# pain7576/ddpg-trucktrailer

Measured on AMD Instinct MI355X. Metric: env-steps/s, higher is better.
Workload: dtype f64

## Files before the change

### ddpg-trucktrailer_amd/_lib.py

```python
import ctypes as C
import os

HERE = os.path.dirname(os.path.abspath(__file__))
LIB_PATH = os.environ.get("TT_LIB_PATH") or os.path.join(HERE, "libttenv.so")

OBS_DIM = 23
MAX_EPISODE_STEPS = 4095
TT_OK, TT_EINVAL, TT_ENOMEM, TT_EHIP, TT_ENODEV = 0, -1, -2, -3, -4
F_JACKKNIFE, F_OUT_OF_MAP, F_MAX_STEPS, F_GOAL_REACHED, F_GOAL_PASSED, F_EXCESSIVE_BACK, F_SUCCESS = (1 << i for i in range(7))
VIOLATIONS = ("none", "jackknife", "jackknife_warning", "major_boundary", "minor_boundary", "past_the_goal",
              "max_step", "excessive_backward")
INFO_ROWS = ("total_reward", "progress_reward", "heading_reward", "orientation_reward", "staged_success",
             "safety_penalty", "exploration_bonus", "final_success_bonus", "backward_penalty", "smoothness_penalty",
             "cumulative_backward", "movement_budget")
NINFO = len(INFO_ROWS)
LOG_COUNTS = ("episodes", "successes", "jackknife", "out_of_map", "max_steps", "goal_reached", "goal_passed",
              "excessive_back", "success_flag")
LOG_DETAIL = 1
LOG_COMPONENTS = INFO_ROWS[1:10]


class TTParams(C.Structure):
    _fields_ = [(n, C.c_double) for n in ("L1", "L2", "hitch_offset", "v1x", "dt", "map_min_x", "map_max_x", "map_min_y",
                                          "map_max_y", "max_steer", "position_threshold", "orientation_threshold",
# ... 127 lines not shown
    "tt_version": (C.c_int, []),
    "tt_last_error": (C.c_char_p, [_P]),
    "tt_params_default": (C.c_int, [_I, C.POINTER(TTParams)]),
    "tt_env_create": (C.c_int, [_I, _I, C.POINTER(TTParams), C.POINTER(_P)]),
    "tt_env_destroy": (C.c_int, [_P]),
    "tt_env_num_envs": (C.c_int, [_P]),
    "tt_env_reset": (C.c_int, [_P, _P, _U64, _P, _P]),
    "tt_env_set_reset_pool": (C.c_int, [_P, _P, _I]),
    "tt_env_set_pose": (C.c_int, [_P, _P, _I, _P, _P, _P, _P, _P]),
    "tt_env_set_attrs": (C.c_int, [_P, _P, _I, _P, _P, _P, _P]),
    "tt_env_set_state": (C.c_int, [_P, _P, _I, _P, _P]),
    "tt_env_get_state": (C.c_int, [_P, _P, _P]),
    "tt_env_set_max_steps": (C.c_int, [_P, _P, _I, _P, _P]),
    "tt_env_set_steps": (C.c_int, [_P, _P, _I, _P, _P]),
    "tt_env_get_episode": (C.c_int, [_P, _P, _P, _P, _P, _P, _P]),
    "tt_env_observe": (C.c_int, [_P, _P, _P, _P]),
    "tt_env_set_step_counter": (C.c_int, [_P, _P]),
    "tt_env_step": (C.c_int, [_P, _P, _P, _P, _P, C.POINTER(TTInfo), _I, _P]),
    "tt_env_step_random": (C.c_int, [_P, _U64, _P, _P, _P, _P, C.POINTER(TTInfo), _I, _P]),
    "tt_env_state_bytes": (C.c_size_t, [_P]),
    "tt_env_export": (C.c_int, [_P, _P, C.POINTER(C.c_uint64 * 4), _P]),
    "tt_env_import": (C.c_int, [_P, _P, C.POINTER(C.c_uint64 * 4), _P]),
    "tt_env_set_episode_log": (C.c_int, [_P, C.c_int64, _P]),
    "tt_env_drain_episode_log": (C.c_int, [_P, _P, _P, _P, _P, _P, _P, _P, _P, _P]),
    "tt_env_episode_log_bytes": (C.c_size_t, [_P]),
    "tt_env_export_episode_log": (C.c_int, [_P, _P, C.POINTER(C.c_uint64 * 2), _P]),
    "tt_env_import_episode_log": (C.c_int, [_P, _P, C.POINTER(C.c_uint64 * 2), _P]),
    "tt_env_set_episode_log2": (C.c_int, [_P, C.c_int64, C.c_uint32, _P]),
    "tt_env_drain_episode_log2": (C.c_int, [_P, _P, _P, _P, _P, _P, _P, _P, _P, _P, _P, _P]),
    "tt_env_rollout_random": (C.c_int, [_P, _I, _U64, _P, _P, _P, _P]),
    "tt_env_profile": (C.c_int, [_P, _I]),
    "tt_env_profile_read": (C.c_int, [_P, C.POINTER(C.c_double), C.POINTER(C.c_int64)]),
    "tt_mlp_split_ws_bytes": (C.c_uint64, []),
    "tt_mlp_split_pack": (C.c_int, [C.POINTER(TTMlpWeights), _I, _P, _P, C.POINTER(TTRingCursor), _P]),
    "tt_mlp_split_pack_and_sample": (C.c_int, [C.POINTER(TTMlpWeights), _I, _P, C.POINTER(TTSampleArgs), C.POINTER(TTRingCursor), _P]),
    "tt_actor_act_ring": (C.c_int, [_I, C.POINTER(TTRingView), C.POINTER(TTMlpWeights), _P, _U64, _U64, _P, C.c_float, C.c_float,
                                    C.c_float, _P, _P]),
    "tt_env_step_ring": (C.c_int, [_P, _P, C.POINTER(TTRingView), _I, _P]),
    "tt_actor_forward": (C.c_int, [_I, _P, C.POINTER(TTMlpWeights), _P, _P]),
    "tt_actor_act": (C.c_int, [_I, _P, C.POINTER(TTMlpWeights), _P, _P, _U64, _U64, _P, C.c_float, C.c_float, C.c_float,
                               _P, _P, _P, _P]),
    "tt_ring_sample": (C.c_int, [_I, _I, _I, _P, _P, _P, _P, _P, _U64, _I, _I, C.POINTER(TTSideBuffer), _P, _P, _P, _P, _P, _P, _P]),
    "tt_critic_forward": (C.c_int, [_I, _P, _P, C.POINTER(TTMlpWeights), _P, _P]),
    "tt_mlp_forward_save": (C.c_int, [_I, _I, _P, _P, C.POINTER(TTMlpWeights), _P, C.POINTER(TTMlpSaved), _P, _P]),
    "tt_mlp_forward_multi": (C.c_int, [_I, _I, C.POINTER(TTFwdJob), _P]),
    "tt_mlp_forward_multi_sampled": (C.c_int, [_I, _I, C.POINTER(TTFwdJob), C.POINTER(TTSampleArgs), _P, _P]),
    "tt_ring_sample_nstep": (C.c_int, [C.POINTER(TTSampleArgs), _I, C.c_float, _P]),
    "tt_mlp_forward_multi_sampled_nstep": (C.c_int, [_I, _I, C.POINTER(TTFwdJob), C.POINTER(TTSampleArgs), _I, C.c_float, _P, _P]),
    "tt_mlp_backward_rows_pair": (C.c_int, [_I, C.c_float, _P, C.POINTER(TTMlpWeights), C.POINTER(TTMlpSaved), C.POINTER(TTMlpBwdWs),
                                            C.POINTER(TTTdInput), _P, C.POINTER(TTMlpWeights), C.POINTER(TTMlpSaved),
                                            C.POINTER(TTMlpBwdWs), C.POINTER(TTImageJob), _P]),
    "tt_mlp_backward_weights": (C.c_int, [_I, _I, _P, _P, C.POINTER(TTMlpSaved), C.POINTER(TTMlpBwdWs), C.POINTER(TTMlpWeights),
                                          _P, _P, C.c_float, _I, _P, _P, _P, _P, _P, C.c_float, C.c_float, C.c_float, C.c_float,
                                          C.c_float, C.c_float, C.POINTER(TTFc2Images), _P, _P]),
    "tt_mlp_actor_tail": (C.c_int, [_I, _P, _P, C.POINTER(TTMlpWeights), _P, _P, C.POINTER(TTMlpSaved), C.POINTER(TTMlpBwdWs),
                                    C.POINTER(TTMlpWeights), C.c_float, _I, _P, _P, _P, _P, _P, C.c_float, C.c_float, C.c_float, C.c_float,
                                    C.c_float, C.c_float, C.POINTER(TTFc2Images), _P, _P, _P, _P]),
    "tt_adam_soft_update": (C.c_int, [_I, _P, _P, _P, _P, _P, _P, _P, C.c_float, C.c_float, C.c_float, C.c_float,
                                      C.c_float, C.c_float, C.POINTER(TTFc2Images), _P, _P]),
    "tt_p2p_create": (C.c_int, [_I, _I, _I, _I, _P, C.POINTER(_P)]),
    "tt_p2p_destroy": (C.c_int, [_P]),
    "tt_p2p_export": (C.c_int, [_P, _P]),
    "tt_p2p_attach": (C.c_int, [_P, _I, _P]),
    "tt_p2p_grad": (_P, [_P, _I]),
    "tt_p2p_reset": (C.c_int, [_P, _P]),
    "tt_p2p_set_timeout": (C.c_int, [_P, C.c_double]),
# ... 90 lines not shown
```

### ddpg-trucktrailer_amd/csrc/ttnet.hip

```cpp
#include <cstdio>
#include <cstdlib>

#include "ttnet_common.h"

using namespace ttnet;

namespace {

constexpr int INP = 24;
constexpr int H2P = 320;
constexpr int NT1 = H1 / 16;
constexpr int NT2 = H2P / 16;
constexpr int BM = 64, WROWS = 16;

using f32x4 = __attribute__((ext_vector_type(4))) float;

template <int CTRL>
__device__ __forceinline__ float dpp_f(float v) {
    return __builtin_bit_cast(float, __builtin_amdgcn_update_dpp(0, __builtin_bit_cast(int, v), CTRL, 0xf, 0xf, true));
}
__device__ __forceinline__ float row_sum16(float v) {
    v += dpp_f<0xB1>(v);
    v += dpp_f<0x4E>(v);
    v += dpp_f<0x141>(v);
// ... 205 lines not shown
        return rc != TT_OK ? rc : split_forward(CRITIC, n, obs, action, w, out, act, stream);
    }
    static bool attr2[64] = {};
    int dev = 0;
    if (hipGetDevice(&dev) != hipSuccess || dev < 0 || dev >= 64) return TT_EHIP;
    if (!attr2[dev]) {
        if (hipFuncSetAttribute(reinterpret_cast<const void *>(&k_mlp_forward_v2<CRITIC>),
                                hipFuncAttributeMaxDynamicSharedMemorySize, V2_LDS_BYTES) != hipSuccess)
            return TT_EHIP;
        attr2[dev] = true;
    }
    hipLaunchKernelGGL((k_mlp_forward_v2<CRITIC>), dim3((n + BM - 1) / BM), dim3(256), V2_LDS_BYTES, stream, n, obs,
                       action, to_weights(w), out, act);
    return hipGetLastError() == hipSuccess ? TT_OK : TT_EHIP;
}

__global__ __launch_bounds__(64) void k_ring_sample(const RingSample R) {
    if ((int)blockIdx.x < R.batch) ring_sample_row(R, blockIdx.x, threadIdx.x);
}

}

extern "C" {

#ifdef TT_STAMPS
int tt_debug_nstamps(unsigned long long *out16) { return ttnet::split_debug_stamps(out16); }
int tt_debug_bstamps(unsigned long long *out, int nblocks) { return ttnet::split_debug_block_stamps(out, nblocks); }
int tt_debug_policy_tiles(unsigned long long *out4096) { return ttnet::split_debug_tiles(out4096); }
int tt_debug_policy_poll(unsigned long long *out4) { return ttnet::split_debug_poll(out4); }
int tt_debug_log_policy(unsigned long long *out, int reset) { return ttnet::split_debug_log(out, reset); }
#endif

uint64_t tt_mlp_split_ws_bytes(void) { return (uint64_t)split_ws_bytes(); }

static RingCursor to_cursor(const tt_ring_cursor *c) {
    return (c && c->cursor && c->k_dev && c->slots > 0)
               ? RingCursor{reinterpret_cast<const long long *>(c->k_dev), c->slots, c->cursor} : RingCursor{nullptr, 0, nullptr};
}

int tt_mlp_split_pack(const tt_mlp_weights *w, int critic, void *ws, int64_t *bump, const tt_ring_cursor *cursor,
                      tt_stream_t stream) {
    if (!ws || !check_ptrs(w, critic != 0)) return TT_EINVAL;
    if (bump && cursor && bump == cursor->k_dev) return TT_EINVAL;
    return split_pack(w, critic != 0, ws, reinterpret_cast<long long *>(bump), to_cursor(cursor), stream);
}

int tt_actor_forward(int n, const float *obs, const tt_mlp_weights *w, float *mu_out, tt_stream_t stream) {
    if (n < 0 || !obs || !mu_out || !check_ptrs(w, false)) return TT_EINVAL;
    if (n == 0) return TT_OK;
    ActArgs act{};
    return launch<false>(n, obs, nullptr, w, mu_out, act, stream);
}

static ActArgs act_args(float *ou_state, const uint8_t *done_prev, float *act_raw, float *act_scaled, const int64_t *step_dev,
                        uint64_t seed, uint64_t step, float theta_dt, float sigma_sqrt_dt, float high) {
    ActArgs act{};
    act.ou = ou_state; act.done_prev = done_prev; act.act_raw = act_raw; act.act_scaled = act_scaled;
    act.step_dev = reinterpret_cast<const long long *>(step_dev);
    act.seed = seed; act.step = step;
    act.decay = 1.0f - theta_dt; act.scale = sigma_sqrt_dt; act.high = high;
    return act;
}

int tt_actor_act(int n, const float *obs, const tt_mlp_weights *w, float *ou_state, const uint8_t *done_prev,
                 uint64_t seed, uint64_t step, const int64_t *step_dev, float theta_dt, float sigma_sqrt_dt, float high,
                 float *mu_out, float *act_raw_out, float *act_scaled_out, tt_stream_t stream) {
// ... 52 lines not shown
```

### ddpg-trucktrailer_amd/csrc/ttnet_common.h

```cpp
#pragma once
#include <hip/hip_runtime.h>

#include <cstdint>

#include "ttenv.h"
#include "ttphilox.h"

namespace ttnet {

constexpr int IN = 23;
constexpr int H1 = 400, H2 = 300;

struct Weights {
    const float *w1, *b1, *g1, *be1;
    const float *w2, *b2, *g2, *be2;
    const float *w3, *b3;
    const float *wa, *ba;
};

struct ActArgs {
    float *ou;
    const uint8_t *done_prev;
    float *act_raw, *act_scaled;
    const long long *step_dev;
// ... 239 lines not shown
    asm volatile("" ::: "memory");
    __syncthreads();
}

__device__ __forceinline__ void await_progress(int *progress, const long long *k_dev) {
    if (!progress) return;
    if (threadIdx.x == 0) {
        const int want = (int)*k_dev;
        if (__hip_atomic_load(progress, __ATOMIC_RELAXED, __HIP_MEMORY_SCOPE_AGENT) - want >= 0) TT_POLL(2);
        else {
            TT_POLL(3);
            const unsigned long long t0 = wall_clock64();
            while (__hip_atomic_load(progress, __ATOMIC_RELAXED, __HIP_MEMORY_SCOPE_AGENT) - want < 0) {
                __builtin_amdgcn_s_sleep(32);
                if (wall_clock64() - t0 > TT_IMAGE_WAIT_TICKS) {
                    mark_gave_up(progress - CUR_PROGRESS, want + 1);
                    break;
                }
            }
            __builtin_amdgcn_fence(__ATOMIC_ACQUIRE, "agent");
            asm volatile("s_waitcnt vmcnt(0)" ::: "memory");
        }
    }
    asm volatile("" ::: "memory");
    __syncthreads();
}

size_t split_ws_bytes();
int split_pack(const tt_mlp_weights *w, bool critic, void *ws, long long *bump, const RingCursor &cur, hipStream_t stream);
int split_pack_and_sample(const tt_mlp_weights *w, bool critic, void *ws, const RingSample &R, const RingCursor &cur,
                          hipStream_t stream);
int split_forward(bool critic, int n, const float *obs, const float *action, const tt_mlp_weights *w, float *out,
                  const ActArgs &act, hipStream_t stream);
#ifdef TT_STAMPS
int split_debug_stamps(unsigned long long *out16);
int split_debug_tiles(unsigned long long *out4096);
int split_debug_poll(unsigned long long *out4);
int split_debug_log(unsigned long long *out, int reset);
int split_debug_block_stamps(unsigned long long *out, int nblocks);
#endif

}
```

### ddpg-trucktrailer_amd/csrc/ttnet_split.hip

```cpp
#include "ttnet_common.h"
#include "ttnet_pack.h"
#include "ttstamps.h"

namespace ttnet {
namespace {

#ifdef TT_STAMPS
__device__ unsigned long long g_nstamps[16];
__device__ unsigned long long g_bstamps[4096 * 8];
#define NSTAMP(i) do { if (threadIdx.x == 0) { const unsigned long long w_ = wall_clock64();                                \
        if (blockIdx.x < 4096) { g_bstamps[blockIdx.x * 8 + (i)] = w_;                                                      \
            if ((i) == 0) g_bstamps[blockIdx.x * 8 + 7] = __builtin_amdgcn_s_getreg((20 << 0) | (0 << 6) | (3 << 11)); }     \
        if (blockIdx.x == 0) { g_nstamps[i] = w_; g_nstamps[8 + i] = clock64(); } } } while (0)
__device__ unsigned long long g_tile[512][4][2];
__device__ TTLog g_log_tile;
#define TSTAMP(round, e) do { if (threadIdx.x == 0 && blockIdx.x < 512 && (round) < 4) g_tile[blockIdx.x][round][e] = wall_clock64(); } while (0)
#else
#define NSTAMP(i) do { } while (0)
#define TSTAMP(round, e) do { } while (0)
#endif

__global__ __launch_bounds__(256) void k_split_pack(const Weights W, const bool critic, unsigned char *__restrict__ ws,
                                                    unsigned char *__restrict__ ws_alt, long long *__restrict__ bump,
                                                    const RingCursor cur) {
    split_pack_body(W, critic, ws, ws_alt, bump, cur, blockIdx.x * 256 + threadIdx.x);
    publish_image(cur, PACK_BLOCKS);
}

__global__ __launch_bounds__(256) void k_pack_and_sample(const Weights W, const bool critic, unsigned char *__restrict__ ws,
                                                         unsigned char *__restrict__ ws_alt, const RingSample R,
                                                         const RingCursor cur) {
    if ((int)blockIdx.x < PACK_BLOCKS) {
// ... 420 lines not shown
                    f32x2 ya = pk_fma(pk(acc2[u][4 * i], acc2[u][4 * i + 1]) * rstd2p, pk(g.x, g.y), pk(be.x, be.y));
                    f32x2 yb = pk_fma(pk(acc2[u][4 * i + 2], acc2[u][4 * i + 3]) * rstd2p, pk(g.z, g.w), pk(be.z, be.w));
                    if (CRITIC) {
                        const float4 wa = vq[u & 1][i][NV - 2], ba = vq[u & 1][i][NV - 1];
                        ya += pk_fma(pk(av, av), pk(wa.x, wa.y), pk(ba.x, ba.y));
                        yb += pk_fma(pk(av, av), pk(wa.z, wa.w), pk(ba.z, ba.w));
                    }
                    dotp = pk_fma(pk(fmaxf(ya[0], 0.f), fmaxf(ya[1], 0.f)), pk(w3.x, w3.y), dotp);
                    dotp = pk_fma(pk(fmaxf(yb[0], 0.f), fmaxf(yb[1], 0.f)), pk(w3.z, w3.w), dotp);
                }
                __builtin_amdgcn_sched_barrier(0);
            }
        }
        const float dot = dotp[0] + dotp[1];
        const float v = dot + __shfl_xor(dot, 32) + lds4(pv1 - 4 * h + VEC_FLOATS).x;
        if (h == 0 && row < n) {
            if (with_noise) finish_row_noise(row, v, out, act, ou_next, araw);
            else finish_row<CRITIC>(row, v, out, act);
        }
        if (first) NSTAMP(5);
#ifdef TT_STAMPS
        TSTAMP(round, 1);
        if (threadIdx.x == 0 && blockIdx.x < 512 && round < 4) tt_log_add(g_log_tile, g_tile[blockIdx.x][round][0], g_tile[blockIdx.x][round][1]);
        ++round;
        if (more_tiles) TSTAMP(round, 0);
#endif
        if (!more_tiles) break;
        tile = next;
        first = false;
    }
    asm volatile("s_waitcnt vmcnt(0)" ::: "memory");
}

}

#ifdef TT_STAMPS
int split_debug_stamps(unsigned long long *out16) {
    return hipMemcpyFromSymbol(out16, HIP_SYMBOL(g_nstamps), sizeof(unsigned long long) * 16) == hipSuccess ? 0 : -3;
}
int split_debug_tiles(unsigned long long *out4096) {
    return hipMemcpyFromSymbol(out4096, HIP_SYMBOL(g_tile), sizeof(unsigned long long) * 512 * 4 * 2) == hipSuccess ? 0 : -3;
}
int split_debug_log(unsigned long long *out, int reset) {
    if (out && hipMemcpyFromSymbol(out, HIP_SYMBOL(g_log_tile), sizeof(TTLog)) != hipSuccess) return -3;
    if (reset) { const unsigned long long z = 0; if (hipMemcpyToSymbol(HIP_SYMBOL(g_log_tile), &z, sizeof(z)) != hipSuccess) return -3; }
    return 0;
}
int split_debug_poll(unsigned long long *out4) {
    return hipMemcpyFromSymbol(out4, HIP_SYMBOL(g_poll), sizeof(unsigned long long) * 4) == hipSuccess ? 0 : -3;
}
int split_debug_block_stamps(unsigned long long *out, int nblocks) {
    return hipMemcpyFromSymbol(out, HIP_SYMBOL(g_bstamps), sizeof(unsigned long long) * 8 * (nblocks < 4096 ? nblocks : 4096)) == hipSuccess ? 0 : -3;
}
#endif

size_t split_ws_bytes() { return (size_t)WS_BYTES; }

int split_pack(const tt_mlp_weights *w, bool critic, void *ws, long long *bump, const RingCursor &cur, hipStream_t stream) {
    unsigned char *alt = ws == w->split_ws ? reinterpret_cast<unsigned char *>(w->split_ws_alt) : nullptr;
    hipLaunchKernelGGL(k_split_pack, dim3(PACK_BLOCKS), dim3(256), 0, stream, to_weights(w), critic,
                       reinterpret_cast<unsigned char *>(ws), alt, bump, cur);
    return hipGetLastError() == hipSuccess ? TT_OK : TT_EHIP;
}

int split_pack_and_sample(const tt_mlp_weights *w, bool critic, void *ws, const RingSample &R, const RingCursor &cur,
                          hipStream_t stream) {
    unsigned char *alt = ws == w->split_ws ? reinterpret_cast<unsigned char *>(w->split_ws_alt) : nullptr;
    hipLaunchKernelGGL(k_pack_and_sample, dim3(PACK_BLOCKS + (R.batch * R.draws + 3) / 4), dim3(256), 0, stream, to_weights(w), critic,
                       reinterpret_cast<unsigned char *>(ws), alt, R, cur);
    return hipGetLastError() == hipSuccess ? TT_OK : TT_EHIP;
}

template <bool CRITIC>
static int launch_split(int n, const float *obs, const float *action, const tt_mlp_weights *w, float *out,
                        const ActArgs &act, hipStream_t stream) {
    static bool attr[64] = {};
    static int cus[64] = {};
    int dev = 0;
    if (hipGetDevice(&dev) != hipSuccess || dev < 0 || dev >= 64) return TT_EHIP;
    if (!attr[dev]) {
        if (hipFuncSetAttribute(reinterpret_cast<const void *>(&k_mlp_split<CRITIC>),
                                hipFuncAttributeMaxDynamicSharedMemorySize, LDS_BYTES) != hipSuccess)
            return TT_EHIP;
        int c = 0;
        if (hipDeviceGetAttribute(&c, hipDeviceAttributeMultiprocessorCount, dev) != hipSuccess || c <= 0) c = 256;
        cus[dev] = c;
        attr[dev] = true;
    }
    const int ntiles = (n + ROWS - 1) / ROWS;
    const int chip = cus[dev];
    int capped = 0;
    if (w->max_workgroups > 0) {
        const int limit = w->max_workgroups;
        capped = ntiles;
        if (w->capped_grids > 0 && (long long)w->capped_grids * limit < ntiles) capped = w->capped_grids * limit;
        const int rounds = (capped + limit - 1) / limit, g = (capped + rounds - 1) / rounds;
        hipLaunchKernelGGL((k_mlp_split<CRITIC>), dim3(g), dim3(256), LDS_BYTES, stream, n, 0, capped, act.cursor, act.step_dev, obs,
                           reinterpret_cast<const unsigned char *>(w->split_ws),
                           reinterpret_cast<const unsigned char *>(w->split_ws_alt), action, out, act);
    }
    if (capped < ntiles) {
        const int rest = ntiles - capped, rounds = (rest + chip - 1) / chip, g = (rest + rounds - 1) / rounds;
        hipLaunchKernelGGL((k_mlp_split<CRITIC>), dim3(g), dim3(256), LDS_BYTES, stream, n, capped, ntiles, act.cursor, act.step_dev, obs,
                           reinterpret_cast<const unsigned char *>(w->split_ws),
                           reinterpret_cast<const unsigned char *>(w->split_ws_alt), action, out, act);
    }
    return hipGetLastError() == hipSuccess ? TT_OK : TT_EHIP;
}

int split_forward(bool critic, int n, const float *obs, const float *action, const tt_mlp_weights *w, float *out,
                  const ActArgs &act, hipStream_t stream) {
    return critic ? launch_split<true>(n, obs, action, w, out, act, stream)
                  : launch_split<false>(n, obs, action, w, out, act, stream);
}

}
```

### ddpg-trucktrailer_amd/fused.py

```python
import contextlib
import ctypes as C
import math

import torch

from ddpg_trucktrailer_amd import _lib as L


def supported(net):
    if not all(hasattr(net, a) for a in ("fc1", "fc2", "bn1", "bn2")) or not (hasattr(net, "mu") or hasattr(net, "q")):
        return False
    return (net.fc1.weight.is_cuda and net.fc1.weight.dtype == torch.float32 and tuple(net.fc1.weight.shape) == (400, 23)
            and tuple(net.fc2.weight.shape) == (300, 400) and net.bn1.eps == 1e-5 and net.bn2.eps == 1e-5)


def pack_and_sample(net, index, sample_args, cursor=None):
    w = packed_weights_of(net, index)
    dev = net.fc2.weight.device
    L.check(L.load().tt_mlp_split_pack_and_sample(C.byref(w), 1 if hasattr(net, "action_value") else 0, C.c_void_p(w.split_ws),
                                                  C.byref(sample_args), C.byref(cursor) if cursor is not None else None,
                                                  L.stream(dev)))


def actor_act_ring(net, ring_view, weights, ou_state, act_scaled, seed, step=0, step_dev=None, theta=0.2, sigma=0.15, dt=1e-2,
                   high=math.pi / 4):
    dev = net.fc2.weight.device
    L.check(L.load().tt_actor_act_ring(int(ring_view.n_envs), C.byref(ring_view), C.byref(weights), L.ptr(ou_state),
                                       int(seed) & (2 ** 64 - 1), int(step), L.ptr(step_dev), float(theta * dt),
                                       float(sigma * math.sqrt(dt)), float(high), L.ptr(act_scaled),
                                       L.stream(dev)))
    return act_scaled


def _fill_weights(net, w):
    head = net.mu if hasattr(net, "mu") else net.q
    for name, t in (("w1", net.fc1.weight), ("b1", net.fc1.bias), ("g1", net.bn1.weight), ("be1", net.bn1.bias),
                    ("w2", net.fc2.weight), ("b2", net.fc2.bias), ("g2", net.bn2.weight), ("be2", net.bn2.bias),
                    ("w3", head.weight), ("b3", head.bias)):
        assert t.is_contiguous()
# ... 62 lines not shown
        w.split_ws = ws


def _stream(t):
    return L.stream(t.device)


def actor_forward(net, obs, out=None):
    n = obs.shape[0]
    out = torch.empty(n, dtype=torch.float32, device=obs.device) if out is None else out
    L.check(L.load().tt_actor_forward(n, L.ptr(obs), C.byref(weights_of(net)), L.ptr(out), _stream(obs)))
    return out.view(n, 1)


def critic_forward(net, obs, action, out=None):
    n = obs.shape[0]
    out = torch.empty(n, dtype=torch.float32, device=obs.device) if out is None else out
    L.check(L.load().tt_critic_forward(n, L.ptr(obs), L.ptr(action), C.byref(weights_of(net)), L.ptr(out), _stream(obs)))
    return out.view(n, 1)


def actor_act(net, obs, ou_state, act_raw, act_scaled, seed, step=0, step_dev=None, done_prev=None, mu_out=None,
              theta=0.2, sigma=0.15, dt=1e-2, high=math.pi / 4, weights=None):
    n = obs.shape[0]
    L.check(L.load().tt_actor_act(n, L.ptr(obs), C.byref(weights if weights is not None else weights_of(net)), L.ptr(ou_state), L.ptr(done_prev),
                                  int(seed) & (2 ** 64 - 1), int(step), L.ptr(step_dev), float(theta * dt),
                                  float(sigma * math.sqrt(dt)), float(high), L.ptr(mu_out), L.ptr(act_raw),
                                  L.ptr(act_scaled), _stream(obs)))
    return act_scaled


def policy_kernel_info(n):
    waves = 4 * ((n + 127) // 128)
    return {"kernel": "k_mlp_split (choose_action for N envs; split-f16; the image's pack launch, ~4 us per step, not included)",
            "mfma_flop": waves * (750 + 78) * 32768.0,
            "note": "f16 MFMA FLOP executed (three f16 products per f32 product block, both layers) over the dense f16/bf16 "
                    "peak; algorithmic_* = the network's useful f32 FLOP"}
```

### include/ttenv.h

```cpp
#ifndef TTENV_H
#define TTENV_H

#include <stddef.h>
#include <stdint.h>

#ifdef __cplusplus
extern "C" {
#endif

#define TT_VERSION 3
#define TT_OBS_DIM 23
#define TT_MAX_EPISODE_STEPS 4095

enum { TT_OK = 0, TT_EINVAL = -1, TT_ENOMEM = -2, TT_EHIP = -3, TT_ENODEV = -4 };

enum {
    TT_F_JACKKNIFE = 1, TT_F_OUT_OF_MAP = 2, TT_F_MAX_STEPS = 4, TT_F_GOAL_REACHED = 8,
    TT_F_GOAL_PASSED = 16, TT_F_EXCESSIVE_BACK = 32, TT_F_SUCCESS = 64
};
#define TT_TERM_SIMV2 0x3F
#define TT_TERM_SIMV1 0x0F

enum {
    TT_V_NONE = 0, TT_V_JACKKNIFE, TT_V_JACKKNIFE_WARNING, TT_V_MAJOR_BOUNDARY, TT_V_MINOR_BOUNDARY,
// ... 104 lines not shown
#define TT_LOG_DETAIL 1
#define TT_LOG_NCOMP 9
int tt_env_set_episode_log2(tt_env *env, int64_t capacity, uint32_t flags, tt_stream_t stream);
int tt_env_drain_episode_log2(tt_env *env, double *ret, int32_t *len, uint8_t *flags, uint8_t *success, int32_t *lane,
                              int64_t *end_step, double *comp, double *start, int64_t *n_out, uint64_t *counts_out,
                              tt_stream_t stream);

int tt_env_rollout_random(tt_env *env, int k_steps, uint64_t policy_seed, float *obs_out, float *reward_sum,
                          int32_t *episodes_done, tt_stream_t stream);

int tt_env_profile(tt_env *env, int max_launches);
int tt_env_profile_read(tt_env *env, double *total_ms, int64_t *launches);

int tt_random_actions(int n, uint64_t seed, uint64_t step, float *out, tt_stream_t stream);

typedef struct tt_mlp_weights {
    const float *w1, *b1, *g1, *be1, *w2, *b2, *g2, *be2, *w3, *b3, *wa, *ba;
    int32_t in_dim, fc1_dims, fc2_dims;
    int32_t capped_grids;
    void *split_ws;
    int32_t ws_packed;
    int32_t max_workgroups;
    void *split_ws_alt;
    void *fc2_img;
} tt_mlp_weights;
uint64_t tt_mlp_fc2_image_bytes(void);
int tt_mlp_fc2_image_pack(const tt_mlp_weights *w, tt_stream_t stream);
typedef struct tt_fc2_images {
    void *net, *target;
} tt_fc2_images;
uint64_t tt_mlp_split_ws_bytes(void);
int tt_mlp_split_pack(const tt_mlp_weights *w, int critic, void *ws, int64_t *bump, const tt_ring_cursor *cursor,
                      tt_stream_t stream);

int tt_actor_forward(int n, const float *obs , const tt_mlp_weights *w, float *mu_out, tt_stream_t stream);

int tt_actor_act(int n, const float *obs, const tt_mlp_weights *w, float *ou_state, const uint8_t *done_prev,
                 uint64_t seed, uint64_t step, const int64_t *step_dev, float theta_dt, float sigma_sqrt_dt, float high,
                 float *mu_out, float *act_raw_out, float *act_scaled_out, tt_stream_t stream);

int tt_actor_act_ring(int n, const tt_ring_view *ring, const tt_mlp_weights *w, float *ou_state, uint64_t seed, uint64_t step,
                      const int64_t *step_dev, float theta_dt, float sigma_sqrt_dt, float high, float *act_scaled_out,
                      tt_stream_t stream);

typedef struct tt_side_buffer {
    const float *obs, *act, *rew, *obs2;
    const uint8_t *done;
    int32_t count, reserved_;
} tt_side_buffer;
int tt_ring_sample(int batch, int n_envs, int slots, const int64_t *k_dev, const float *obs, const float *act,
                   const float *rew, const uint8_t *done, uint64_t seed, int reserve, int lag, const tt_side_buffer *side,
                   float *s_out, float *a_out, float *r_out, float *s2_out, uint8_t *d_out, int32_t *idx_out,
                   tt_stream_t stream);

typedef struct tt_sample_args {
    int32_t batch, n_envs, slots, reserve;
    const int64_t *k_dev;
    const float *obs, *act, *rew;
    const uint8_t *done;
    uint64_t seed;
    const tt_side_buffer *side;
    float *s_out, *a_out, *r_out, *s2_out;
    uint8_t *d_out;
    int32_t *idx_out;
    int32_t lag;
    int32_t draws;
// ... 214 lines not shown
```

Measured before the change: 807.5 million.

## Add shadowed policy MLP kernel that hides noise, LN1 sums and next-tile loads under MFMAs

```diff
diff --git a/ddpg-trucktrailer_amd/_lib.py b/ddpg-trucktrailer_amd/_lib.py
--- a/ddpg-trucktrailer_amd/_lib.py
+++ b/ddpg-trucktrailer_amd/_lib.py
@@ -183,6 +183,7 @@
     "tt_env_profile": (C.c_int, [_P, _I]),
     "tt_env_profile_read": (C.c_int, [_P, C.POINTER(C.c_double), C.POINTER(C.c_int64)]),
     "tt_mlp_split_ws_bytes": (C.c_uint64, []),
+    "tt_mlp_split_variant": (C.c_int, [_I]),
     "tt_mlp_split_pack": (C.c_int, [C.POINTER(TTMlpWeights), _I, _P, _P, C.POINTER(TTRingCursor), _P]),
     "tt_mlp_split_pack_and_sample": (C.c_int, [C.POINTER(TTMlpWeights), _I, _P, C.POINTER(TTSampleArgs), C.POINTER(TTRingCursor), _P]),
     "tt_actor_act_ring": (C.c_int, [_I, C.POINTER(TTRingView), C.POINTER(TTMlpWeights), _P, _U64, _U64, _P, C.c_float, C.c_float,
diff --git a/ddpg-trucktrailer_amd/csrc/ttnet.hip b/ddpg-trucktrailer_amd/csrc/ttnet.hip
--- a/ddpg-trucktrailer_amd/csrc/ttnet.hip
+++ b/ddpg-trucktrailer_amd/csrc/ttnet.hip
@@ -261,6 +261,7 @@
 #endif
 
 uint64_t tt_mlp_split_ws_bytes(void) { return (uint64_t)split_ws_bytes(); }
+int tt_mlp_split_variant(int v) { return split_variant(v); }
 
 static RingCursor to_cursor(const tt_ring_cursor *c) {
     return (c && c->cursor && c->k_dev && c->slots > 0)
diff --git a/ddpg-trucktrailer_amd/csrc/ttnet_common.h b/ddpg-trucktrailer_amd/csrc/ttnet_common.h
--- a/ddpg-trucktrailer_amd/csrc/ttnet_common.h
+++ b/ddpg-trucktrailer_amd/csrc/ttnet_common.h
@@ -295,6 +295,7 @@
                           hipStream_t stream);
 int split_forward(bool critic, int n, const float *obs, const float *action, const tt_mlp_weights *w, float *out,
                   const ActArgs &act, hipStream_t stream);
+int split_variant(int v);
 #ifdef TT_STAMPS
 int split_debug_stamps(unsigned long long *out16);
 int split_debug_tiles(unsigned long long *out4096);
diff --git a/ddpg-trucktrailer_amd/csrc/ttnet_shadow.h b/ddpg-trucktrailer_amd/csrc/ttnet_shadow.h
--- /dev/null
+++ b/ddpg-trucktrailer_amd/csrc/ttnet_shadow.h
@@ -0,0 +1,490 @@
+#ifndef TT_SHADOW_NOISE
+#define TT_SHADOW_NOISE 1
+#endif
+#ifndef TT_SHADOW_LN1
+#define TT_SHADOW_LN1 1
+#endif
+#ifndef TT_SHADOW_EPI
+#define TT_SHADOW_EPI 1
+#endif
+#ifndef TT_SHADOW_OBS
+#define TT_SHADOW_OBS 0
+#endif
+constexpr bool SH_NOISE = TT_SHADOW_NOISE != 0, SH_LN1 = TT_SHADOW_LN1 != 0, SH_EPI = TT_SHADOW_EPI != 0, SH_OBS = TT_SHADOW_OBS != 0;
+constexpr int OBS_LOADS = S1 * 8 + 2;
+constexpr bool step_has_no_job(const int s) {
+    for (int u = 0; u < T2; ++u) if (l2_job(s, u) != JOB_NONE) return false;
+    return true;
+}
+constexpr bool step_waits(const int s) { return s >= 1 && s + 1 < STEPS; }
+static_assert(step_has_no_job(STEPS - 1) && OBS_LOADS + 1 <= 3 * T2,
+              "the next tile's loads take free job slots of the last k16 step only (slot 0 forms their address)");
+static_assert(!step_waits(STEPS - 1), "no counted wait may follow the first of the next tile's loads");
+
+template <bool CRITIC>
+__global__ __launch_bounds__(256, 1) void k_mlp_split_shadow(const int n, const int tile0, const int tile_end,
+                                                             int *__restrict__ cursor_e, const long long *__restrict__ step_e,
+                                                             const float *__restrict__ obs,
+                                                             const unsigned char *__restrict__ ws,
+                                                             const unsigned char *__restrict__ ws_alt,
+                                                             const float *__restrict__ action, float *__restrict__ out,
+                                                             const ActArgs act) {
+    extern __shared__ __attribute__((aligned(16))) unsigned char lds_raw[];
+    const float *p1_s = reinterpret_cast<const float *>(lds_raw + RING_BYTES);
+    const int tid = threadIdx.x, lane = tid & 63;
+    const int wave = __builtin_amdgcn_readfirstlane(tid >> 6);
+    const int r = lane & 31, h = lane >> 5;
+    using lds_f = const __attribute__((address_space(3))) float;
+    using v4 = __attribute__((ext_vector_type(4))) float;
+    auto lds4 = [](lds_f *q) -> float4 {
+        const v4 t = *(const __attribute__((address_space(3))) v4 *)q;
+        return make_float4(t[0], t[1], t[2], t[3]);
+    };
+    lds_f *pv1_0 = (lds_f *)(p1_s + 4 * h);
+    LdsBases LB0;
+    LB0.b0 = (lds_b *)lds_raw + lane * 16;
+    LB0.b1 = LB0.b0 + 65536;
+    LB0.b2 = LB0.b0 + 131072;
+    const EpochPair epochs = await_image_early(cursor_e);
+    const long long kstep = cursor_e ? *step_e : 0;
+    const bool odd = act.cursor && (kstep & 1);
+    const bool local = act.cursor && act.ring_slots > 0;
+    const int slot_t = !local ? 0 : ((unsigned long long)kstep >> 32) == 0ull ? (int)((unsigned)kstep % (unsigned)act.ring_slots)
+                                                                             : (int)(kstep % act.ring_slots);
+    const float *obs_base = local ? obs + (size_t)slot_t * act.ring_n * IN : obs;
+    const unsigned lds_base0 = (unsigned)(uintptr_t)(__attribute__((address_space(3))) unsigned char *)lds_raw;
+    auto dma_piece = [&](const unsigned char *base, const unsigned voff, const unsigned lds_wave, const unsigned dst_const)
+                         __attribute__((always_inline)) {
+        unsigned keep;
+        asm volatile("s_mov_b32 %0, m0\n\ts_add_u32 m0, %3, %4\n\ts_nop 0\n\tglobal_load_lds_dwordx4 %1, %2\n\ts_mov_b32 m0, %0"
+                     : "=&s"(keep) : "v"(voff), "s"(base), "s"(lds_wave), "s"(dst_const) : "memory", "scc");
+    };
+    const unsigned voff_w2 = lane * 16 + wave * 5120 + WS_W2;
+    const unsigned voff_w1 = lane * 16 + wave * 1024 + WS_W1;
+    const unsigned voff_vec = lane * 16 + wave * (VEC_PIECES / 4) * 1024 + WS_VEC;
+    const unsigned ldsw_w2_0 = lds_base0 + wave * 5120, ldsw_w1_0 = lds_base0 + W1_OFF + wave * 1024;
+    auto issue_fc1_piece = [&](const unsigned char *w, const unsigned ldsw_w1, const int i) __attribute__((always_inline)) {
+        dma_piece(w, voff_w1 + i * 4096, ldsw_w1, i * 4096);
+    };
+    auto issue_step_piece = [&](const unsigned char *w, const unsigned ldsw_w2, const int s, const int i) __attribute__((always_inline)) {
+        dma_piece(w, voff_w2 + s * CHUNK_BYTES + i * 1024, ldsw_w2, (s % RING) * CHUNK_BYTES + i * 1024);
+    };
+    float xo[S1][8];
+    float ou_pre = 0.f;
+    unsigned dp_pre = 0u;
+    const bool with_noise = !CRITIC && act.ou != nullptr;
+    const uint8_t *dprev = act.done_prev;
+    float *araw = act.act_raw;
+    auto load_obs = [&](const int tile) __attribute__((always_inline)) {
+        const int row = tile * ROWS + wave * WROWS + r;
+        const int rowc = row < n ? row : n - 1;
+        const float *orow = obs_base + (size_t)rowc * IN;
+#pragma unroll
+        for (int s = 0; s < S1; ++s)
+#pragma unroll
+            for (int j = 0; j < 8; ++j) {
+                const int k = 16 * s + 8 * h + j;
+                xo[s][j] = orow[k < IN ? k : IN - 1];
+            }
+        if (with_noise) {
+            ou_pre = act.ou[rowc];
+            dp_pre = dprev ? (unsigned)dprev[rowc] : 0u;
+        }
+    };
+
+    NSTAMP(0);
+    int tile = tile0 + (int)blockIdx.x;
+    if (tile >= tile_end) return;
+    if (local) {
+        const int sl = act.ring_slots;
+        const int slot_prev = slot_t == 0 ? sl - 1 : slot_t - 1;
+        dprev = kstep > 0 ? act.done_prev + (size_t)slot_prev * act.ring_n : nullptr;
+        araw = act.act_raw + (size_t)slot_t * act.ring_n;
+    }
+    if (!act.cursor || local) load_obs(tile);
+    await_image(act.cursor, act.step_dev, epochs);
+    const unsigned char *wsl = (odd && ws_alt) ? ws_alt : ws;
+    if (act.cursor && !local) {
+        obs_base = resolve_obs(act, obs);
+        const int *c = cursor_of(act);
+        dprev = c[3] ? act.done_prev + (size_t)c[2] * act.ring_n : nullptr;
+        araw = act.act_raw + (size_t)c[0] * act.ring_n;
+        load_obs(tile);
+    }
+    const unsigned long long noise_step = act.step + (act.step_dev ? (unsigned long long)*act.step_dev : 0ull);
+    if (act.cursor && tile0 == 0 && blockIdx.x == 0 && tid == 0)
+        __hip_atomic_store(act.cursor + CUR_PROGRESS, (int)(kstep + 1), __ATOMIC_RELAXED, __HIP_MEMORY_SCOPE_AGENT);
+    if (act.cursor && tile0 == 0 && blockIdx.x == 0 && tid < 4) {
+        const int sl = act.ring_slots;
+        act.cursor[tid] = !local ? cursor_of(act)[tid]
+                                 : (tid == 0 ? slot_t : tid == 1 ? (slot_t + 1 == sl ? 0 : slot_t + 1)
+                                                      : tid == 2 ? (slot_t == 0 ? sl - 1 : slot_t - 1) : (kstep > 0 ? 1 : 0));
+    }
+#pragma unroll
+    for (int i = 0; i < W1_WAVE_PIECES; ++i) issue_fc1_piece(wsl, ldsw_w1_0, i);
+#pragma unroll
+    for (int i = 0; i < VEC_PIECES / 4; ++i)
+        dma_piece(wsl, voff_vec + i * 1024, lds_base0 + RING_BYTES + wave * (VEC_PIECES / 4) * 1024, i * 1024);
+    bool first = true;
+#ifdef TT_STAMPS
+    int round = 0;
+    if (threadIdx.x == 0 && blockIdx.x < 512) for (int q = 0; q < 4; ++q) g_tile[blockIdx.x][q][0] = g_tile[blockIdx.x][q][1] = 0ull;
+    if (threadIdx.x == 0 && blockIdx.x < 512) g_tile[blockIdx.x][0][0] = wall_clock64();
+#endif
+
+#pragma unroll 1
+    for (;;) {
+        const unsigned char *wsl_cur = wsl;
+        unsigned ldsw_w2 = ldsw_w2_0, ldsw_w1 = ldsw_w1_0;
+        LdsBases LB = LB0;
+        lds_f *pv1 = pv1_0;
+        asm volatile("" : "+s"(wsl_cur), "+s"(ldsw_w2), "+s"(ldsw_w1), "+v"(LB.b0), "+v"(LB.b1), "+v"(LB.b2), "+v"(pv1));
+        lds_f *pv2 = pv1 + 2 * H1P;
+        const int row = tile * ROWS + wave * WROWS + r;
+#pragma unroll
+        for (int s = 0; s < S1; ++s)
+#pragma unroll
+            for (int j = 0; j < 8; ++j) {
+                const int k = 16 * s + 8 * h + j;
+                xo[s][j] = k < IN ? (row < n ? xo[s][j] : 0.f) : (k == IN ? 1.f : 0.f);
+            }
+        float ou_next = 0.f;
+        auto restarts = [&]() __attribute__((always_inline)) { return dp_pre != 0u && with_noise && dprev != nullptr; };
+        if (!SH_NOISE && with_noise) ou_next = ou_advance(row < n ? row : n - 1, ou_pre, restarts(), act, noise_step);
+        uint32_t nc0 = 0u, nc1 = 0u, nc2 = 0u, nc3 = 0u, nhi0 = 0u, nlo0 = 0u;
+        float nu1 = 0.f, nu2 = 0.f;
+        auto noise_chunk = [&](const int c) __attribute__((always_inline)) {
+            if (c == 0) {
+                nc0 = (uint32_t)(row < n ? row : n - 1); nc1 = (uint32_t)noise_step; nc2 = (uint32_t)(noise_step >> 32); nc3 = 0x0A5Eu;
+                asm volatile("" : "+v"(nc0));
+            } else if (c <= 20) {
+                const int rd = (c - 1) >> 1;
+                if ((c - 1) & 1) {
+                    const uint32_t k0 = (uint32_t)act.seed + (uint32_t)rd * 0x9E3779B9u, k1 = (uint32_t)(act.seed >> 32) + (uint32_t)rd * 0xBB67AE85u;
+                    const uint32_t hi1 = __umulhi(0xCD9E8D57u, nc2), lo1 = 0xCD9E8D57u * nc2;
+                    const uint32_t n0 = hi1 ^ nc1 ^ k0, n2 = nhi0 ^ nc3 ^ k1;
+                    nc0 = n0; nc1 = lo1; nc2 = n2; nc3 = nlo0;
+                    asm volatile("" : "+v"(nc0), "+v"(nc1), "+v"(nc2));
+                } else {
+                    nhi0 = __umulhi(0xD2511F53u, nc0); nlo0 = 0xD2511F53u * nc0;
+                    asm volatile("" : "+v"(nhi0), "+v"(nlo0));
+                }
+            } else if (c == 21) {
+                nu1 = ((float)(nc0 >> 8) + 0.5f) * (1.f / 16777216.f);
+                nu2 = ((float)(nc1 >> 8) + 0.5f) * (1.f / 16777216.f);
+                asm volatile("" : "+v"(nu1), "+v"(nu2));
+            } else if (c == 22) {
+                nu1 = logf(nu1);
+                asm volatile("" : "+v"(nu1));
+            } else if (c == 23) {
+                nu1 = sqrtf(-2.f * nu1);
+                asm volatile("" : "+v"(nu1));
+            } else if (c == 24) {
+                nu2 = cosf(6.28318530717958647692f * nu2);
+                asm volatile("" : "+v"(nu2));
+            } else {
+                const float nrm = nu1 * nu2;
+                ou_next = fmaf(restarts() ? 0.f : ou_pre, act.decay, act.scale * nrm);
+                asm volatile("" : "+v"(ou_next));
+            }
+        };
+        constexpr int NOISE_CHUNKS = 26;
+        static_assert(NOISE_CHUNKS <= S1 * T1, "one chunk of the noise per product of layer 1");
+        uint4 xb[S1][2];
+#pragma unroll
+        for (int s = 0; s < S1; ++s) {
+            uint32_t ph[4], pm[4];
+#pragma unroll
+            for (int p = 0; p < 4; ++p) split2(xo[s][2 * p] * SX, xo[s][2 * p + 1] * SX, ph[p], pm[p]);
+            xb[s][0] = make_uint4(ph[0], ph[1], ph[2], ph[3]);
+            xb[s][1] = make_uint4(pm[0], pm[1], pm[2], pm[3]);
+        }
+        asm volatile("s_waitcnt vmcnt(0)" ::: "memory");
+        __builtin_amdgcn_s_barrier();
+        if (first) NSTAMP(1);
+
+#define SB __builtin_amdgcn_sched_barrier(0)
+        f32x16 acc1[T1];
+        f32x2 sp1 = pk(0.f, 0.f);
+        auto ln1_sum = [&](const int t, const int v) __attribute__((always_inline)) {
+            sp1 += pk(acc1[t][v], acc1[t][v + 1]) + pk(acc1[t][v + 2], acc1[t][v + 3]);
+        };
+        {
+            auto w1_frag = [&](const int q, const int plane) __attribute__((always_inline)) {
+                return lds_frag(LB, W1_OFF + (((q % S1) * T1 + q / S1) * 2 + plane) * 1024);
+            };
+            const unsigned char *wsl_1 = wsl_cur;
+            asm volatile("" : "+s"(wsl_1));
+            uint4 a0h = w1_frag(0, 0), a0m = w1_frag(0, 1), a1h = w1_frag(1, 0), a1m = w1_frag(1, 1), a2h = a0h, a2m = a0m;
+            SB;
+#pragma unroll
+            for (int q = 0; q < S1 * T1; ++q) {
+                const int t = q / S1, s = q % S1;
+                if (s == 0) {
+#pragma unroll
+                    for (int v = 0; v < 16; ++v) acc1[t][v] = 0.f;
+                }
+                acc1[t] = mfma_f16(a0m, xb[s][0], acc1[t]); SB;
+                if (q + 2 < S1 * T1) a2h = w1_frag(q + 2, 0);
+                if (SH_NOISE && !CRITIC && q < NOISE_CHUNKS) noise_chunk(q);
+                SB;
+                acc1[t] = mfma_f16(a0h, xb[s][1], acc1[t]); SB;
+                if (q + 2 < S1 * T1) a2m = w1_frag(q + 2, 1);
+                if (SH_LN1 && q >= 4) {
+                    ln1_sum((q - 4) >> 1, 8 * (q & 1));
+                    ln1_sum((q - 4) >> 1, 8 * (q & 1) + 4);
+                    asm volatile("" : "+v"(sp1));
+                }
+                SB;
+                acc1[t] = mfma_f16(a0h, xb[s][0], acc1[t]); SB;
+                if (q < 10) { if (first) issue_step_piece(wsl_1, ldsw_w2, q / 5, q % 5); }
+                else if (q < 20) issue_step_piece(wsl_1, ldsw_w2, 2 + (q - 10) / 5, q % 5);
+                SB;
+                a0h = a1h; a0m = a1m; a1h = a2h; a1m = a2m;
+            }
+        }
+        if (first) NSTAMP(2);
+        uint32_t hb[STEPS][4], mb[STEPS][4];
+        f32x2 nmean, rstdp;
+        {
+#pragma unroll
+            for (int t = SH_LN1 ? T1 - 2 : 0; t < T1; ++t)
+#pragma unroll
+                for (int v = 0; v < (t == T1 - 1 ? 8 : 16); v += 4) ln1_sum(t, v);
+            const f32x2 sp = sp1;
+            const float s = sp[0] + sp[1];
+            const float mean = (s + __shfl_xor(s, 32)) * (1.f / H1);
+            nmean = pk(-mean, -mean);
+            f32x2 ssp = pk(0.f, 0.f);
+#pragma unroll
+            for (int t = 0; t < T1; ++t)
+#pragma unroll
+                for (int v = 0; v < (t == T1 - 1 ? 8 : 16); v += 2) {
+                    const f32x2 d = pk(acc1[t][v], acc1[t][v + 1]) + nmean;
+                    ssp = pk_fma(d, d, ssp);
+                }
+            const float ss = ssp[0] + ssp[1];
+            const float var = (ss + __shfl_xor(ss, 32)) * (1.f / H1) * (UNSCALE * UNSCALE);
+            const float rstd = rsqrtf(var + 1e-5f) * UNSCALE;
+            rstdp = pk(rstd, rstd);
+        }
+        constexpr int GROUPS = 2 * STEPS;
+        float4 gq[2], bq[2];
+        f32x2 ya, yb;
+        float y0, y1, y2, y3;
+        auto ln_read = [&](const int G) __attribute__((always_inline)) {
+            gq[G & 1] = lds4(pv1 + 8 * G);
+            bq[G & 1] = lds4(pv1 + H1P + 8 * G);
+        };
+        auto ln_chunk = [&](const int G, const int k) __attribute__((always_inline)) {
+            const int t = G >> 2, i = G & 3, st = G >> 1, e = 2 * (G & 1);
+            const float4 g = gq[G & 1], be = bq[G & 1];
+            if (k == 0) ya = pk_fma((pk(acc1[t][4 * i], acc1[t][4 * i + 1]) + nmean) * rstdp, pk(g.x, g.y), pk(be.x, be.y));
+            if (k == 1) yb = pk_fma((pk(acc1[t][4 * i + 2], acc1[t][4 * i + 3]) + nmean) * rstdp, pk(g.z, g.w), pk(be.z, be.w));
+            if (k == 2) {
+                y0 = fmaxf(ya[0], 0.f); y1 = fmaxf(ya[1], 0.f); y2 = fmaxf(yb[0], 0.f); y3 = fmaxf(yb[1], 0.f);
+                if (G + 1 < GROUPS) ln_read(G + 1);
+            }
+            if (k == 3) split2(y0, y1, hb[st][e], mb[st][e]);
+            if (k == 4) split2(y2, y3, hb[st][e + 1], mb[st][e + 1]);
+        };
+        ln_read(0);
+#pragma unroll
+        for (int G = 0; G < 4; ++G)
+#pragma unroll
+            for (int k = 0; k < 5; ++k) ln_chunk(G, k);
+
+        if (first) NSTAMP(3);
+        f32x16 acc2[T2];
+#pragma unroll
+        for (int u = 0; u < T2; ++u)
+#pragma unroll
+            for (int v = 0; v < 16; ++v) acc2[u][v] = 0.f;
+        f32x2 s2p = pk(0.f, 0.f);
+        float4 bq2[2][4];
+        auto ldb = [&](const int u, float4 (&b)[4]) __attribute__((always_inline)) {
+#pragma unroll
+            for (int i = 0; i < 4; ++i) b[i] = lds4(pv2 + 32 * u + 8 * i);
+        };
+        auto ep1_group = [&](const int u, const int i) __attribute__((always_inline)) {
+            const float4 b = bq2[u & 1][i];
+            const f32x2 xa = pk_fma(pk(acc2[u][4 * i], acc2[u][4 * i + 1]), pk(UNSCALE, UNSCALE), pk(b.x, b.y));
+            const f32x2 xb2 = pk_fma(pk(acc2[u][4 * i + 2], acc2[u][4 * i + 3]), pk(UNSCALE, UNSCALE), pk(b.z, b.w));
+            acc2[u][4 * i] = xa[0]; acc2[u][4 * i + 1] = xa[1]; acc2[u][4 * i + 2] = xb2[0]; acc2[u][4 * i + 3] = xb2[1];
+            s2p += xa + xb2;
+        };
+        const int next = tile + (int)gridDim.x;
+        const bool more_tiles = next < tile_end;
+        const float *orow_n = obs_base;
+        const float *ou_n = obs_base;
+        const uint8_t *dp_n = reinterpret_cast<const uint8_t *>(obs_base);
+        auto next_load = [&](const int i) __attribute__((always_inline)) {
+            if (i == 0) {
+                const int row_n = (more_tiles ? next : tile) * ROWS + wave * WROWS + r;
+                const int rowc = row_n < n ? row_n : n - 1;
+                orow_n = obs_base + (size_t)rowc * IN;
+                const bool use_dp = with_noise && dprev != nullptr;
+                ou_n = with_noise ? act.ou + rowc : orow_n;
+                dp_n = use_dp ? dprev + rowc : reinterpret_cast<const uint8_t *>(orow_n);
+            } else if (i <= S1 * 8) {
+                const int s = (i - 1) >> 3, j = (i - 1) & 7, k = 16 * s + 8 * h + j;
+                xo[s][j] = orow_n[k < IN ? k : IN - 1];
+            } else if (!CRITIC && i == S1 * 8 + 1) {
+                ou_pre = *ou_n;
+            } else if (!CRITIC && i == S1 * 8 + 2) {
+                dp_pre = (unsigned)*dp_n;
+            }
+        };
+        auto last_step_job = [&](const int u, const int k) __attribute__((always_inline)) {
+            if (SH_OBS && 3 * u + k <= OBS_LOADS) next_load(3 * u + k);
+            if (SH_EPI) {
+                if (u == 1 && k == 0) ldb(0, bq2[0]);
+                if (u >= 2) {
+                    const int e = u - 2;
+                    if (k == 0) { ldb(e + 1, bq2[(e + 1) & 1]); ep1_group(e, 0); }
+                    if (k == 1) ep1_group(e, 1);
+                    if (k == 2) { ep1_group(e, 2); ep1_group(e, 3); }
+                    asm volatile("" : "+v"(s2p));
+                }
+            }
+        };
+        asm volatile("s_waitcnt vmcnt(10)" ::: "memory");
+        __builtin_amdgcn_s_barrier();
+        uint4 c0h = lds_frag(LB, 0), c0m = lds_frag(LB, 1024), c1h = lds_frag(LB, 2048), c1m = lds_frag(LB, 3072), c2h = c0h, c2m = c0m;
+        SB;
+        auto l2_step = [&](const int s) __attribute__((always_inline)) {
+            const uint4 vh = make_uint4(hb[s][0], hb[s][1], hb[s][2], hb[s][3]), vm = make_uint4(mb[s][0], mb[s][1], mb[s][2], mb[s][3]);
+            const int slot = (s % RING) * CHUNK_BYTES, nslot = ((s + 1) % RING) * CHUNK_BYTES;
+            const unsigned char *wsl_s = wsl_cur;
+            unsigned lds_s = ldsw_w2, lds1_s = ldsw_w1;
+            asm volatile("" : "+s"(wsl_s), "+s"(lds_s));
+            if (s >= TAIL0 && s < TAIL0 + 3) asm volatile("" : "+s"(lds1_s));
+#pragma unroll
+            for (int u = 0; u < T2; ++u) {
+                if (u == T2 / 2 && step_waits(s)) {
+                    switch (L2S.mid[s]) {
+                        case 20: asm volatile("s_waitcnt vmcnt(20)" ::: "memory"); break;
+                        default: asm volatile("s_waitcnt vmcnt(18)" ::: "memory"); break;
+                    }
+                    __builtin_amdgcn_s_barrier();
+                    SB;
+                }
+                const bool more = u + 2 < T2 || s + 1 < STEPS;
+                const int nx = u + 2 < T2 ? slot + (u + 2) * 2048 : nslot + (u + 2 - T2) * 2048;
+                acc2[u] = mfma_f16(c0h, vm, acc2[u]); SB;
+                if (more) c2h = lds_frag(LB, nx);
+                if (s + 2 < STEPS) ln_chunk(2 * (s + 2) + u / 5, u % 5);
+                if (s == STEPS - 1) last_step_job(u, 0);
+                SB;
+                acc2[u] = mfma_f16(c0m, vh, acc2[u]); SB;
+                if (more) c2m = lds_frag(LB, nx + 1024);
+                if (s == STEPS - 1) last_step_job(u, 1);
+                SB;
+                acc2[u] = mfma_f16(c0h, vh, acc2[u]); SB;
+                if (s == STEPS - 1) last_step_job(u, 2);
+                {
+                    const int j = L2S.job[s][u];
+                    const bool f1 = j >= JOB_FC1 && j < JOB_NEXT;
+                    const int st = j >= JOB_NEXT ? j - JOB_NEXT : j, i1 = j - JOB_FC1;
+                    if (j != JOB_NONE)
+                        dma_piece(wsl_s, f1 ? voff_w1 + i1 * 4096 : voff_w2 + st * CHUNK_BYTES + l2_piece(u) * 1024, f1 ? lds1_s : lds_s,
+                                  f1 ? i1 * 4096 : (st % RING) * CHUNK_BYTES + l2_piece(u) * 1024);
+                }
+                SB;
+                c0h = c1h; c0m = c1m; c1h = c2h; c1m = c2m;
+            }
+        };
+#pragma unroll
+        for (int s = 0; s < 2; ++s) l2_step(s);
+#pragma unroll
+        for (int s = 2; s < TAIL0; ++s) l2_step(s);
+#pragma unroll
+        for (int s = TAIL0; s < STEPS; ++s) l2_step(s);
+#undef SB
+
+        if (first) NSTAMP(4);
+        if (!SH_OBS && more_tiles) load_obs(next);
+        {
+            constexpr int U0 = SH_EPI ? T2 - 2 : 0;
+            if (!SH_EPI) ldb(0, bq2[0]);
+#pragma unroll
+            for (int u = U0; u < T2; ++u) {
+                if (u + 1 < T2) ldb(u + 1, bq2[(u + 1) & 1]);
+                __builtin_amdgcn_sched_barrier(0);
+#pragma unroll
+                for (int i = 0; i < 4; ++i) ep1_group(u, i);
+                __builtin_amdgcn_sched_barrier(0);
+            }
+        }
+        const float s2 = s2p[0] + s2p[1];
+        const float mean2 = (s2 + __shfl_xor(s2, 32)) * (1.f / H2);
+        const f32x2 nmean2 = pk(-mean2, -mean2);
+        f32x2 ss2p = pk(0.f, 0.f);
+#pragma unroll
+        for (int u = 0; u < T2; ++u)
+#pragma unroll
+            for (int i = 0; i < 4; ++i) {
+                const bool real = 32 * u + 8 * i + 4 * h < H2;
+                const f32x2 keep = real ? pk(1.f, 1.f) : pk(0.f, 0.f);
+#pragma unroll
+                for (int j = 0; j < 4; j += 2) {
+                    const f32x2 d = pk(acc2[u][4 * i + j], acc2[u][4 * i + j + 1]) + nmean2;
+                    acc2[u][4 * i + j] = d[0]; acc2[u][4 * i + j + 1] = d[1];
+                    const f32x2 dk = (32 * u + 8 * i + 4 < H2) ? d : d * keep;
+                    ss2p = pk_fma(dk, dk, ss2p);
+                }
+            }
+        const float ss2 = ss2p[0] + ss2p[1];
+        const float rstd2 = rsqrtf((ss2 + __shfl_xor(ss2, 32)) * (1.f / H2) + 1e-5f);
+        const f32x2 rstd2p = pk(rstd2, rstd2);
+        const float av = (CRITIC && row < n) ? action[row] : 0.f;
+        f32x2 dotp = pk(0.f, 0.f);
+        {
+            constexpr int NV = CRITIC ? 5 : 3;
+            float4 vq[2][4][NV];
+            auto ldv = [&](const int u, float4 (&v)[4][NV]) {
+#pragma unroll
+                for (int i = 0; i < 4; ++i)
+#pragma unroll
+                    for (int q = 0; q < NV; ++q) v[i][q] = lds4(pv2 + (q + 1) * H2P + 32 * u + 8 * i);
+            };
+            ldv(0, vq[0]);
+#pragma unroll
+            for (int u = 0; u < T2; ++u) {
+                if (u + 1 < T2) ldv(u + 1, vq[(u + 1) & 1]);
+                __builtin_amdgcn_sched_barrier(0);
+#pragma unroll
+                for (int i = 0; i < 4; ++i) {
+                    const float4 g = vq[u & 1][i][0], be = vq[u & 1][i][1], w3 = vq[u & 1][i][2];
+                    f32x2 ya = pk_fma(pk(acc2[u][4 * i], acc2[u][4 * i + 1]) * rstd2p, pk(g.x, g.y), pk(be.x, be.y));
+                    f32x2 yb = pk_fma(pk(acc2[u][4 * i + 2], acc2[u][4 * i + 3]) * rstd2p, pk(g.z, g.w), pk(be.z, be.w));
+                    if (CRITIC) {
+                        const float4 wa = vq[u & 1][i][NV - 2], ba = vq[u & 1][i][NV - 1];
+                        ya += pk_fma(pk(av, av), pk(wa.x, wa.y), pk(ba.x, ba.y));
+                        yb += pk_fma(pk(av, av), pk(wa.z, wa.w), pk(ba.z, ba.w));
+                    }
+                    dotp = pk_fma(pk(fmaxf(ya[0], 0.f), fmaxf(ya[1], 0.f)), pk(w3.x, w3.y), dotp);
+                    dotp = pk_fma(pk(fmaxf(yb[0], 0.f), fmaxf(yb[1], 0.f)), pk(w3.z, w3.w), dotp);
+                }
+                __builtin_amdgcn_sched_barrier(0);
+            }
+        }
+        const float dot = dotp[0] + dotp[1];
+        const float v = dot + __shfl_xor(dot, 32) + lds4(pv1 - 4 * h + VEC_FLOATS).x;
+        if (h == 0 && row < n) {
+            if (with_noise) finish_row_noise(row, v, out, act, ou_next, araw);
+            else finish_row<CRITIC>(row, v, out, act);
+        }
+        if (first) NSTAMP(5);
+#ifdef TT_STAMPS
+        TSTAMP(round, 1);
+        if (threadIdx.x == 0 && blockIdx.x < 512 && round < 4) tt_log_add(g_log_tile, g_tile[blockIdx.x][round][0], g_tile[blockIdx.x][round][1]);
+        ++round;
+        if (more_tiles) TSTAMP(round, 0);
+#endif
+        if (!more_tiles) break;
+        tile = next;
+        first = false;
+    }
+    asm volatile("s_waitcnt vmcnt(0)" ::: "memory");
+}
diff --git a/ddpg-trucktrailer_amd/csrc/ttnet_split.hip b/ddpg-trucktrailer_amd/csrc/ttnet_split.hip
--- a/ddpg-trucktrailer_amd/csrc/ttnet_split.hip
+++ b/ddpg-trucktrailer_amd/csrc/ttnet_split.hip
@@ -1,3 +1,7 @@
+#include <atomic>
+#include <cstdlib>
+#include <cstring>
+
 #include "ttnet_common.h"
 #include "ttnet_pack.h"
 #include "ttstamps.h"
@@ -484,6 +488,8 @@
     asm volatile("s_waitcnt vmcnt(0)" ::: "memory");
 }
 
+#include "ttnet_shadow.h"
+
 }
 
 #ifdef TT_STAMPS
@@ -521,6 +527,19 @@
     hipLaunchKernelGGL(k_pack_and_sample, dim3(PACK_BLOCKS + (R.batch * R.draws + 3) / 4), dim3(256), 0, stream, to_weights(w), critic,
                        reinterpret_cast<unsigned char *>(ws), alt, R, cur);
     return hipGetLastError() == hipSuccess ? TT_OK : TT_EHIP;
+}
+
+int split_variant(const int v) {
+    static std::atomic<int> variant{-1};
+    int cur = variant.load(std::memory_order_relaxed);
+    if (cur < 0) {
+        const char *e = std::getenv("TT_POLICY_KERNEL");
+        const int init = (e && std::strcmp(e, "pinned") == 0) ? TT_POLICY_PINNED : TT_POLICY_SHADOW;
+        variant.compare_exchange_strong(cur, init, std::memory_order_relaxed);
+        cur = variant.load(std::memory_order_relaxed);
+    }
+    if (v == TT_POLICY_SHADOW || v == TT_POLICY_PINNED) cur = variant.exchange(v, std::memory_order_relaxed);
+    return cur;
 }
 
 template <bool CRITIC>
@@ -530,10 +549,13 @@
     static int cus[64] = {};
     int dev = 0;
     if (hipGetDevice(&dev) != hipSuccess || dev < 0 || dev >= 64) return TT_EHIP;
+    using Kernel = void (*)(int, int, int, int *, const long long *, const float *, const unsigned char *, const unsigned char *,
+                            const float *, float *, ActArgs);
+    const Kernel kernel = split_variant(-1) == TT_POLICY_PINNED ? &k_mlp_split<CRITIC> : &k_mlp_split_shadow<CRITIC>;
     if (!attr[dev]) {
-        if (hipFuncSetAttribute(reinterpret_cast<const void *>(&k_mlp_split<CRITIC>),
-                                hipFuncAttributeMaxDynamicSharedMemorySize, LDS_BYTES) != hipSuccess)
-            return TT_EHIP;
+        for (const Kernel k : {Kernel(&k_mlp_split<CRITIC>), Kernel(&k_mlp_split_shadow<CRITIC>)})
+            if (hipFuncSetAttribute(reinterpret_cast<const void *>(k), hipFuncAttributeMaxDynamicSharedMemorySize, LDS_BYTES) != hipSuccess)
+                return TT_EHIP;
         int c = 0;
         if (hipDeviceGetAttribute(&c, hipDeviceAttributeMultiprocessorCount, dev) != hipSuccess || c <= 0) c = 256;
         cus[dev] = c;
@@ -547,13 +569,13 @@
         capped = ntiles;
         if (w->capped_grids > 0 && (long long)w->capped_grids * limit < ntiles) capped = w->capped_grids * limit;
         const int rounds = (capped + limit - 1) / limit, g = (capped + rounds - 1) / rounds;
-        hipLaunchKernelGGL((k_mlp_split<CRITIC>), dim3(g), dim3(256), LDS_BYTES, stream, n, 0, capped, act.cursor, act.step_dev, obs,
+        hipLaunchKernelGGL(kernel, dim3(g), dim3(256), LDS_BYTES, stream, n, 0, capped, act.cursor, act.step_dev, obs,
                            reinterpret_cast<const unsigned char *>(w->split_ws),
                            reinterpret_cast<const unsigned char *>(w->split_ws_alt), action, out, act);
     }
     if (capped < ntiles) {
         const int rest = ntiles - capped, rounds = (rest + chip - 1) / chip, g = (rest + rounds - 1) / rounds;
-        hipLaunchKernelGGL((k_mlp_split<CRITIC>), dim3(g), dim3(256), LDS_BYTES, stream, n, capped, ntiles, act.cursor, act.step_dev, obs,
+        hipLaunchKernelGGL(kernel, dim3(g), dim3(256), LDS_BYTES, stream, n, capped, ntiles, act.cursor, act.step_dev, obs,
                            reinterpret_cast<const unsigned char *>(w->split_ws),
                            reinterpret_cast<const unsigned char *>(w->split_ws_alt), action, out, act);
     }
diff --git a/ddpg-trucktrailer_amd/fused.py b/ddpg-trucktrailer_amd/fused.py
--- a/ddpg-trucktrailer_amd/fused.py
+++ b/ddpg-trucktrailer_amd/fused.py
@@ -5,6 +5,13 @@
 import torch
 
 from ddpg_trucktrailer_amd import _lib as L
+
+
+POLICY_SHADOW, POLICY_PINNED = 0, 1
+
+
+def policy_kernel(variant=None):
+    return int(L.load().tt_mlp_split_variant(-1 if variant is None else int(variant)))
 
 
 def supported(net):
@@ -133,7 +140,8 @@
 
 def policy_kernel_info(n):
     waves = 4 * ((n + 127) // 128)
-    return {"kernel": "k_mlp_split (choose_action for N envs; split-f16; the image's pack launch, ~4 us per step, not included)",
+    name = "k_mlp_split" if L.load().tt_mlp_split_variant(-1) == POLICY_PINNED else "k_mlp_split_shadow"
+    return {"kernel": name + " (choose_action for N envs; split-f16; the image's pack launch, ~4 us per step, not included)",
             "mfma_flop": waves * (750 + 78) * 32768.0,
             "note": "f16 MFMA FLOP executed (three f16 products per f32 product block, both layers) over the dense f16/bf16 "
                     "peak; algorithmic_* = the network's useful f32 FLOP"}
diff --git a/include/ttenv.h b/include/ttenv.h
--- a/include/ttenv.h
+++ b/include/ttenv.h
@@ -160,6 +160,10 @@
 uint64_t tt_mlp_split_ws_bytes(void);
 int tt_mlp_split_pack(const tt_mlp_weights *w, int critic, void *ws, int64_t *bump, const tt_ring_cursor *cursor,
                       tt_stream_t stream);
+
+#define TT_POLICY_SHADOW 0
+#define TT_POLICY_PINNED 1
+int tt_mlp_split_variant(int v);
 
 int tt_actor_forward(int n, const float *obs , const tt_mlp_weights *w, float *mu_out, tt_stream_t stream);
 
```

Measured after the change: 808.5 million, median of 2. Within noise of the previous version (+0.1%).
